# zju-vipa/ProtoPFormer

Hardware: AMD Instinct MI355X
Metric: images/sec train step, deit_small+2000 protos, bs256, 1/2/4/8 MI355X (higher is better)
Workload: dtype bf16; 1 GPU; deit_small_patch16_224, synthetic 224x224, 2000x384 prototypes, 200 classes, k=81, batch 256/GPU (BASELINE.json configs[2]), train step = fwd+CE+PPC+bwd+allreduce+AdamW+EMA, DropPath 0.1; blocks after the token reservation run compacted on the 1+k reserved rows (equal to the masked full-length blocks to bf16 rounding); bf16 backbone: the reserved tokens differ from the fp32 reference's in ~2-3 % o; global_batch=256, parallelism=dp1

## Files before the change

### include/ppf_hip.h

```cpp
#ifndef PPF_HIP_H
#define PPF_HIP_H

#include <stddef.h>
#include <stdint.h>

#ifdef __cplusplus
extern "C" {
#endif

typedef struct ihipStream_t* ppf_stream_t;

#define PPF_ERR_SHAPE (-1)
#define PPF_ERR_ALIGN (-2)
#define PPF_ERR_ARG (-3)

#define PPF_ABI_VERSION 10

const char* ppf_last_error(void);
int ppf_abi_version(void);
int ppf_device_info(int* cu_count, int* clock_mhz, char* name, int name_len);
int ppf_stream_arm(ppf_stream_t stream, int on);
int ppf_stream_wait_stream(ppf_stream_t dst, ppf_stream_t src);
int64_t ppf_stream_mark(ppf_stream_t stream);
int ppf_stream_wait_mark(ppf_stream_t stream, int64_t ticket);

int ppf_gemm_bf16(const void* A, const void* B, void* C, int M, int N, int K, int lda, int ldb, int ldc, int trans_a,
                  int trans_b, int epi, const float* bias, const float* res, int ldres, const float* rowscale,
                  int rows_per_group, const float* colscale, const void* aux_in, void* aux_out, int ldaux, float* colsum,
                  float alpha, void* workspace, size_t workspace_bytes, ppf_stream_t stream);
size_t ppf_gemm_workspace_bytes(int M, int N, int K);

int ppf_gemm_test_force_g224(int force);

int ppf_gemm_probe(int enable);
int ppf_gemm_probe_read(double* ms_total, int64_t* launches, double* flops, double* bytes);

int ppf_path_probe(int enable);
int ppf_path_probe_read(int tag, double* ms_total, int64_t* launches, double* flops, double* bytes);

int ppf_gemm_bf16_batched(const void* A, const void* B, void* C, int M, int N, int K, int lda, int ldb, int ldc, int trans_a,
                          int trans_b, int out_f32, float alpha, int batch_outer, int batch_inner, int64_t sa_o, int64_t sa_i,
                          int64_t sb_o, int64_t sb_i, int64_t sc_o, int64_t sc_i, int kpad, ppf_stream_t stream);

int ppf_layernorm_bwd_f32(const float* dy, const float* x, const int* row_map, const float* w, const float* dres_in, float* dx_out, float* dw, float* db,
                          int rows, int D, float eps, ppf_stream_t stream);
int ppf_ew_bwd_f32(int kind, const float* a, const float* b, float* out, const float* rowscale, int rows_per_group, int M, int N, ppf_stream_t stream);
int ppf_colsum_f32(const float* in, float* out, int M, int N, ppf_stream_t stream);
int ppf_attn_bwd_f32(const float* qkv, const float* dout, const float* policy, float* dqkv, float* scratch, int B, int H, int N, int D, int self_keep,
                     int eps_n, ppf_stream_t stream);
int ppf_th_attn_bwd_f32(const float* qkv, const float* dout, const float* wl, const float* bl, const float* ww, const float* bw, float* dqkv,
                        float* dwl, float* dbl, float* dww, float* dbw, int B, int H, int N, int D, ppf_stream_t stream);
int ppf_class_attn_bwd_f32(const float* q, const float* k, const float* v, const float* policy, const float* dout, float* dq, float* dk, float* dv,
                           int B, int H, int N1, int D, ppf_stream_t stream);

int ppf_rowgemm_supported(int D, int K, int rows_per_tile);
int ppf_rowgemm_bf16(const void* A, const void* B, int M, int D, int K, int lda, int ldb, int rows_per_tile, const float* bias, void* out,
                     ppf_stream_t stream);
int ppf_rowgemm_resid_ln(const void* A, const void* B, int M, int D, int K, int lda, int ldb, int rows_per_tile, const float* bias,
                         const float* res, float* xout, const float* rowscale, int rows_per_group, const float* colscale, void* aux_out,
                         const float* ln_w, const float* ln_b, void* ln_out, float* ln_mean, float* ln_rstd, float eps, ppf_stream_t stream);
int ppf_rowgemm_lnbwd(const void* A, const void* B, int M, int D, int K, int lda, int ldb, int rows_per_tile, const float* x, const float* mean,
                      const float* rstd, const float* w, const float* dres_in, float* dx_out, void* cast_out, const float* rowscale,
                      int rows_per_group, const float* colscale, const void* branch, float* partial, size_t partial_bytes, ppf_stream_t stream);
int ppf_rowgemm_colsum(const float* partial, int tiles, int D, int nparts, float* dw, float* db, float* dg, ppf_stream_t stream);
int ppf_transpose_bf16_batched(const void* src, void* dst, const void* desc_i64, int n, int total_tiles, ppf_stream_t stream);

int ppf_layernorm_fwd(const float* x, const int* row_map, const float* w, const float* b, void* y, float* mean, float* rstd,
                      int rows, int D, float eps, ppf_stream_t stream);
int ppf_layernorm_bwd(const void* dy, const float* x, const int* row_map, const float* w, const float* mean, const float* rstd,
                      const float* dres_in, float* dx_out, float* dw, float* db, void* cast_out, const float* rowscale,
                      int rows_per_group, const float* colscale, float* dbias_next, const void* branch, float* dcolscale,
                      int rows, int D, float* partial, size_t partial_bytes, ppf_stream_t stream);
int ppf_layernorm_bwd_blocks(int rows);
int ppf_layernorm_bwd_reduce(const float* partial, int rows, int D, float* dw, float* db, float* dbias_next, float* dcolscale,
                             ppf_stream_t stream);

int ppf_attn_fwd(const void* qkv, void* out, const float* policy, float* rowmax, float* zinv, int B, int H, int N, int D,
                 int self_keep, int eps_n, ppf_stream_t stream);
int ppf_attn_fwd_hm_supported(int H, int N, int D);
int ppf_attn_fwd_hm(const void* qkv, void* out, const float* policy, float* rowmax, float* zinv, float* headmean, int NP, int B, int H, int N,
                    int D, int self_keep, int eps_n, ppf_stream_t stream);
int ppf_attn_headmean(const void* qkv, const float* policy, const float* rowmax, const float* zinv, float* headmean, int NP,
                      int B, int H, int N, int D, int self_keep, int eps_n, ppf_stream_t stream);
int ppf_attn_bwd(const void* qkv, const void* out, const void* dout, void* dqkv, const float* policy, const float* rowmax,
                 const float* zinv, float* delta, int B, int H, int N, int D, int self_keep, int eps_n, ppf_stream_t stream);

int ppf_th_scores(const void* qkv, const float* wl, const float* bl, float* sp, int B, int H, int N, int D, int NP, ppf_stream_t stream);
int ppf_th_dwl(const void* qkv, const float* ds_prime, float* dwl, int B, int H, int N, int D, int NP, ppf_stream_t stream);
int ppf_th_softmax_mix(float* sp, void* a16, float* hm, const float* ww, const float* bw, int B, int H, int N, int NP, int NPK,
                       ppf_stream_t stream);
int ppf_th_softmax_bwd(const float* prob, float* da, void* ds16, const float* ww, const float* wl, float* dww, float* dbw, float* dbl,
                       int B, int H, int N, int NP, int NPK, ppf_stream_t stream);
int ppf_th_fused_supported(int H, int N, int D);
int ppf_th_fwd(const void* qkv, const float* wl, const float* bl, const float* ww, const float* bw, void* a16, float* hm, float* rowmax,
               float* zinv, void* out, int B, int H, int N, int D, int NP, int NPK, ppf_stream_t stream);
size_t ppf_th_bwd_partial_floats(int B, int H, int N);
int ppf_th_bwd(const void* qkv, const void* dout, const float* wl, const float* bl, const float* ww, const float* rowmax, const float* zinv,
               void* ds16, float* partial, int B, int H, int N, int D, int NPK, ppf_stream_t stream);
int ppf_th_param_reduce(const float* partial, int B, int H, int N, float* dww, float* dbw, float* dbl, float* dwl, ppf_stream_t stream);
int ppf_th_grads_supported(int H, int N, int D);
int ppf_th_grads(const void* qkv, const void* dout, const void* ds16, const void* a16, void* dqkv, int B, int H, int N, int D, int NPK,
                 ppf_stream_t stream);
int ppf_class_attn_fwd(const void* q, const void* k, const void* v, const float* policy, float* attn, float* zinv, float* rowmean,
                       void* out, int B, int H, int N1, int D, ppf_stream_t stream);
int ppf_class_attn_bwd(const void* q, const void* k, const void* v, const float* attn, const float* zinv, const void* dout, void* dq,
                       void* dk, void* dv, int B, int H, int N1, int D, ppf_stream_t stream);
int ppf_merge3_cast(const float* a, const float* b, const float* cq, void* out, int rows, int D, int N1, ppf_stream_t stream);

int ppf_rollout_threshold(const float* hm_layer, int B, int N, int NP, int kdrop, void* thr_out_u32, ppf_stream_t stream);
int ppf_rollout(const float* hm, int64_t layer_stride, int L, int B, int N, int NP, const float* init_rows, int n_init, int lead,
                int kdrop, int kdrop_init, float identity, int k, const void* thr_u32, float* cls_attn, int* idx, float* policy,
                ppf_stream_t stream);
int ppf_topk_sorted(const float* scores, int B, int n, int k, int* idx, ppf_stream_t stream);

int ppf_proto_fwd(const float* tok, int64_t stride_b, int t0, int T, const float* protos, int B, int P, int Dp, int act_kind,
// ... 122 lines not shown
```

### protopformer_amd/csrc/gemm_bf16.hip

```cpp
#include "ppf_common.h"
#include "ppf_hip.h"
#include "gemm_common.h"
#include <cstdlib>
#include <type_traits>

namespace {
using namespace ppfg;

constexpr int BM = 128, BN = 128, BK = 64, NTHREADS = 256;
constexpr int TILE_BYTES = BM * BK * 2;
constexpr int STAGE_LD = 68;
constexpr int STAGE_BYTES = 4 * 32 * STAGE_LD * 4;


__device__ __forceinline__ int lds_off_mode0(int r, int c16) { return lds_row_off(r, c16); }
template <int ROWS>
__device__ __forceinline__ int lds_off_mode1(int kc, int col) {
    return kc * (ROWS * 2) + ((((col >> 5) ^ (kc & 3))) << 6) + ((col & 31) << 1);
}

typedef uint32_t u32x4 __attribute__((ext_vector_type(4)));

template <bool T, int ROWS, int NTHR = NTHREADS>
struct TileIO {
    static constexpr int NLD = ROWS * 8 / NTHR;
    static constexpr int RPP = NTHR / 8;
    static constexpr int CPR = ROWS / 8;
    static constexpr int KPP = NTHR / CPR;
    static __device__ __forceinline__ unsigned gload(u32x4 (&reg)[NLD], const bf16_t* __restrict__ X, int ld, int R, int row0,
                                                     int k0, int kend, int tid, int kpad) {
        unsigned mask = 0;
        if constexpr (!T) {
            const int c16 = tid & 7, rb = tid >> 3;
            const bool kok = kpad ? (k0 + c16 * 8) < kend : (k0 + c16 * 8 + 8) <= kend;
            const int kk = kok ? k0 + c16 * 8 : 0;
#pragma unroll
            for (int i = 0; i < NLD; ++i) {
                const int r = row0 + rb + RPP * i;
                const bf16_t* src = X + (size_t)min(r, R - 1) * ld + kk;
                reg[i] = *reinterpret_cast<const u32x4*>(src);
                mask |= (kok && r < R) ? (1u << i) : 0u;
            }
        } else {
            const int c16 = tid % CPR, kb = tid / CPR;
            const int col = row0 + c16 * 8;
            const bool cok = kpad ? col < R : (col + 8) <= R;
            const int cc = cok ? col : 0;
#pragma unroll
            for (int i = 0; i < NLD; ++i) {
                const int kc = k0 + kb + KPP * i;
                const bf16_t* src = X + (size_t)min(kc, kend - 1) * ld + cc;
                reg[i] = *reinterpret_cast<const u32x4*>(src);
                mask |= (cok && kc < kend) ? (1u << i) : 0u;
            }
        }
        return mask;
    }
    static __device__ __forceinline__ void sstore(const u32x4 (&reg)[NLD], unsigned mask, unsigned char* tile, int tid) {
        const u32x4 zero = {0u, 0u, 0u, 0u};
        if constexpr (!T) {
            const int c16 = tid & 7, rb = tid >> 3;
#pragma unroll
            for (int i = 0; i < NLD; ++i)
                *reinterpret_cast<u32x4*>(tile + lds_off_mode0(rb + RPP * i, c16)) = ((mask >> i) & 1u) ? reg[i] : zero;
        } else {
            const int c16 = tid % CPR, kb = tid / CPR;
#pragma unroll
            for (int i = 0; i < NLD; ++i)
                *reinterpret_cast<u32x4*>(tile + lds_off_mode1<ROWS>(kb + KPP * i, c16 * 8)) = ((mask >> i) & 1u) ? reg[i] : zero;
        }
    }
    static __device__ __forceinline__ bf16x8 frag(const unsigned char* tile, int rbase, int ks, int lane) {
        if constexpr (!T) {
            return *reinterpret_cast<const bf16x8*>(tile + lds_off_mode0(rbase + (lane & 31), ks * 2 + (lane >> 5)));
        } else {
            typedef __attribute__((address_space(3))) bf16x4 lds_bf16x4;
            const int s = lane & 15, g16 = (lane >> 4) & 1, h = lane >> 5;
            const int col = rbase + 16 * g16 + 4 * (s & 3);
            const int kc = ks * 16 + 8 * h + (s >> 2);
            bf16x4 lo = __builtin_amdgcn_ds_read_tr16_b64_v4bf16((lds_bf16x4*)(tile + lds_off_mode1<ROWS>(kc, col)));
            bf16x4 hi = __builtin_amdgcn_ds_read_tr16_b64_v4bf16((lds_bf16x4*)(tile + lds_off_mode1<ROWS>(kc + 4, col)));
            return __builtin_shufflevector(lo, hi, 0, 1, 2, 3, 4, 5, 6, 7);
        }
    }
};


template <int EPI>
__device__ __forceinline__ void epilogue_rows(const GemmParams& p, const float* stage, int mbase, int nbase, int lane) {
    if (EpiWide<EPI>::value && ((p.ldc | p.ldaux) & 7) == 0) {
        const int col = (lane & 7) * 8;
        const int n = nbase + col;
        if (n + 8 <= p.N) {
            const EpiCols8 cc = epi_load_cols8<EPI>(p, n, true);
            EpiRow8 rr[4];
#pragma unroll
            for (int pass = 0; pass < 4; ++pass) {
                const int m = mbase + pass * 8 + (lane >> 3);
                rr[pass] = epi_load_row8<EPI>(p, m, n, m < p.M);
            }
#pragma unroll
            for (int pass = 0; pass < 4; ++pass) {
                const int r = pass * 8 + (lane >> 3);
                const int m = mbase + r;
                const float4 a = *reinterpret_cast<const float4*>(stage + r * STAGE_LD + col);
                const float4 b = *reinterpret_cast<const float4*>(stage + r * STAGE_LD + col + 4);
                if (m < p.M) epi_store8<EPI>(p, m, n, a, b, cc, rr[pass]);
            }
        } else if (n < p.N) {
            const EpiCols cc = epi_load_cols<EPI>(p, n, true);
#pragma unroll
            for (int pass = 0; pass < 4; ++pass) {
                const int r = pass * 8 + (lane >> 3);
                const int m = mbase + r;
                if (m < p.M) {
                    const EpiRow rr = epi_load_row<EPI>(p, m, n, true);
                    const float4 v = *reinterpret_cast<const float4*>(stage + r * STAGE_LD + col);
                    epi_store<EPI>(p, m, n, v.x, v.y, v.z, v.w, cc, rr);
                }
            }
        }
    } else {
        const int col = (lane & 15) * 4;
        const int n = nbase + col;
        const EpiCols cc = epi_load_cols<EPI>(p, n, n < p.N);
        EpiRow rr[8];
#pragma unroll
        for (int pass = 0; pass < 8; ++pass) {
            const int m = mbase + pass * 4 + (lane >> 4);
            rr[pass] = epi_load_row<EPI>(p, m, n, m < p.M && n < p.N);
        }
#pragma unroll
        for (int pass = 0; pass < 8; ++pass) {
            const int r = pass * 4 + (lane >> 4);
            const int m = mbase + r;
            const float4 v = *reinterpret_cast<const float4*>(stage + r * STAGE_LD + col);
            if (m < p.M && n < p.N) epi_store<EPI>(p, m, n, v.x, v.y, v.z, v.w, cc, rr[pass]);
        }
    }
}

struct KSlice { int kbeg, kend; };
__device__ __forceinline__ KSlice k_slice(int K, int nsplit, int zslice) {
    const int kchunk = (((K + nsplit - 1) / nsplit) + BK - 1) / BK * BK;
    const int kbeg = zslice * kchunk;
    return {kbeg, min(K, kbeg + kchunk)};
}

template <int EPI, int MT>
__device__ __forceinline__ void strip_epilogue(const GemmParams& p, const f32x16 (&acc)[2][MT], int mi, unsigned char* smem, int wave, int lane,
                                               int mbase, int nbase) {
    const int h = lane >> 5;
    float* stage = reinterpret_cast<float*>(smem) + wave * (32 * STAGE_LD);
#pragma unroll
    for (int ni = 0; ni < 2; ++ni)
#pragma unroll
        for (int g = 0; g < 4; ++g)
            *reinterpret_cast<float4*>(stage + (lane & 31) * STAGE_LD + 32 * ni + 8 * g + 4 * h) =
                make_float4(acc[ni][mi][4 * g], acc[ni][mi][4 * g + 1], acc[ni][mi][4 * g + 2], acc[ni][mi][4 * g + 3]);
    __builtin_amdgcn_wave_barrier();
    epilogue_rows<EPI>(p, stage, mbase, nbase, lane);
    __builtin_amdgcn_wave_barrier();
}

__device__ __forceinline__ void store_partial_colsum(const GemmParams& p, int m, float v) {
    p.ws[p.zslice * ((size_t)p.M * p.N + (size_t)p.cs_parts * p.M) + (size_t)p.M * p.N + m] = v;
}

template <bool TA, bool TB, int EPI, bool COLSUM>
__global__ __launch_bounds__(NTHREADS, 3) void gemm_kernel(const GemmParams p_) {
    constexpr int PD = 1, MT = 2;
    extern __shared__ __attribute__((aligned(16))) unsigned char smem[];
    constexpr int TBM = 64 * MT;
    constexpr int A_BYTES = TBM * BK * 2;
    using IOA = TileIO<TA, TBM>;
    using IOB = TileIO<TB, BN>;
    const int tid = threadIdx.x, lane = tid & 63, wave = tid >> 6;
    const int wm = (wave & 1) * (32 * MT), wn = (wave >> 1) * 64;

    const int tiles_n = (p_.N + BN - 1) / BN;
    const int tiles = tiles_n * ((p_.M + TBM - 1) / TBM);
    const int vid_all = xcd_remap(blockIdx.x, gridDim.x);
    const int zslice = vid_all / tiles, vid = vid_all - zslice * tiles;
    const int m0 = (vid / tiles_n) * TBM, n0 = (vid % tiles_n) * BN;
    GemmParams p = p_;
    p.zslice = zslice;
    if (gridDim.y > 1) {
        const int bo = blockIdx.y / p.batch_inner, bi = blockIdx.y % p.batch_inner;
        p.A += bo * p.sa_o + bi * p.sa_i;
        p.B += bo * p.sb_o + bi * p.sb_i;
        const long long co = bo * p.sc_o + bi * p.sc_i;
        p.C = (EPI == EPI_BF16) ? (void*)(reinterpret_cast<bf16_t*>(p.C) + co) : (void*)(reinterpret_cast<float*>(p.C) + co);
    }

    const auto [kbeg, kend] = k_slice(p.K, p.nsplit, zslice);
    if (kbeg >= kend) return;
    const int nk = (kend - kbeg + BK - 1) / BK;

    u32x4 ra[PD][IOA::NLD], rb[PD][IOB::NLD];
    unsigned ma[PD], mb[PD];
    f32x16 acc[2][MT];
#pragma unroll
    for (int i = 0; i < 2; ++i)
#pragma unroll
        for (int j = 0; j < MT; ++j)
#pragma unroll
            for (int r = 0; r < 16; ++r) acc[i][j][r] = 0.f;
    f32x16 accs[MT];
    if constexpr (COLSUM) {
#pragma unroll
        for (int j = 0; j < MT; ++j)
#pragma unroll
            for (int r = 0; r < 16; ++r) accs[j][r] = 0.f;
    }
    const bool do_colsum = COLSUM && p.colsum != nullptr && n0 == 0 && wn == 0;
    unsigned char* tA = smem;
    unsigned char* tB = smem + A_BYTES;

#pragma unroll
    for (int st = 0; st < PD; ++st) {
        const int k0 = min(kbeg + st * BK, kbeg + (nk - 1) * BK);
        ma[st] = IOA::gload(ra[st], p.A, p.lda, p.M, m0, k0, kend, tid, p.kpad);
        mb[st] = IOB::gload(rb[st], p.B, p.ldb, p.N, n0, k0, kend, tid, p.kpad);
    }
    IOA::sstore(ra[0], ma[0], tA, tid);
    IOB::sstore(rb[0], mb[0], tB, tid);
    __syncthreads();

    for (int kt0 = 0; kt0 < nk; kt0 += PD) {
#pragma unroll
        for (int u = 0; u < PD; ++u) {
            const int kt = kt0 + u;
            if (kt >= nk) break;
            {
                const int k0 = kbeg + min(kt + PD, nk - 1) * BK;
                ma[u] = IOA::gload(ra[u], p.A, p.lda, p.M, m0, k0, kend, tid, p.kpad);
                mb[u] = IOB::gload(rb[u], p.B, p.ldb, p.N, n0, k0, kend, tid, p.kpad);
            }
#pragma unroll
            for (int ks = 0; ks < BK / 16; ++ks) {
                bf16x8 fa[MT], fb[2];
#pragma unroll
                for (int i = 0; i < MT; ++i) fa[i] = IOA::frag(tA, wm + 32 * i, ks, lane);
#pragma unroll
                for (int i = 0; i < 2; ++i) fb[i] = IOB::frag(tB, wn + 32 * i, ks, lane);
#pragma unroll
                for (int ni = 0; ni < 2; ++ni)
#pragma unroll
                    for (int mi = 0; mi < MT; ++mi)
                        acc[ni][mi] = __builtin_amdgcn_mfma_f32_32x32x16_bf16(fb[ni], fa[mi], acc[ni][mi], 0, 0, 0);
                if constexpr (COLSUM) {
                    if (do_colsum) {
                        bf16x8 ones;
#pragma unroll
                        for (int e = 0; e < 8; ++e) ones[e] = (__bf16)1.0f;
#pragma unroll
                        for (int mi = 0; mi < MT; ++mi)
                            accs[mi] = __builtin_amdgcn_mfma_f32_32x32x16_bf16(ones, fa[mi], accs[mi], 0, 0, 0);
                    }
                }
            }
            __syncthreads();
            if (kt + 1 < nk) {
                IOA::sstore(ra[(u + 1) % PD], ma[(u + 1) % PD], tA, tid);
                IOB::sstore(rb[(u + 1) % PD], mb[(u + 1) % PD], tB, tid);
            }
            __syncthreads();
        }
    }

#pragma unroll
    for (int mi = 0; mi < MT; ++mi) {
        strip_epilogue<EPI>(p, acc, mi, smem, wave, lane, m0 + wm + 32 * mi, n0 + wn);
        if constexpr (COLSUM) {
            const int m = m0 + wm + 32 * mi + (lane & 31);
            if (do_colsum && (lane >> 5) == 0 && m < p.M) {
                if constexpr (EPI == EPI_PARTIAL) store_partial_colsum(p, m, accs[mi][0]);
                else unsafeAtomicAdd(p.colsum + m, accs[mi][0]);
            }
        }
    }
}

template <int WMW, int WNW, bool COLSUM>
__global__ __launch_bounds__(64 * WMW * WNW, 1) void wgrad8_kernel(const GemmParams p_) {
    extern __shared__ __attribute__((aligned(16))) unsigned char smem[];
    constexpr int NTHR = 64 * WMW * WNW, TBM = 64 * WMW, TBN = 64 * WNW;
    using IOA = TileIO<true, TBM, NTHR>;
    using IOB = TileIO<true, TBN, NTHR>;
    const int tid = threadIdx.x, lane = tid & 63;
    const int wave = __builtin_amdgcn_readfirstlane(tid >> 6);
    const int wm = (wave % WMW) * 64, wn = (wave / WMW) * 64;
    const int tiles_n = (p_.N + TBN - 1) / TBN;
    const int tiles = tiles_n * ((p_.M + TBM - 1) / TBM);
    const int vid_all = xcd_remap(blockIdx.x, gridDim.x);
    const int zslice = vid_all / tiles, vid = vid_all - zslice * tiles;
    const int m0 = (vid / tiles_n) * TBM, n0 = (vid % tiles_n) * TBN;
    GemmParams p = p_;
    p.zslice = zslice;
    const auto [kbeg, kend] = k_slice(p.K, p.nsplit, zslice);
    if (kbeg >= kend) return;
    const int nk = (kend - kbeg + BK - 1) / BK;

    u32x4 ra[IOA::NLD], rb[IOB::NLD];
    unsigned ma, mb;
    f32x16 acc[2][2];
#pragma unroll
    for (int i = 0; i < 2; ++i)
#pragma unroll
        for (int j = 0; j < 2; ++j)
#pragma unroll
            for (int r = 0; r < 16; ++r) acc[i][j][r] = 0.f;
    f32x16 accs[2];
    if constexpr (COLSUM) {
#pragma unroll
        for (int j = 0; j < 2; ++j)
#pragma unroll
            for (int r = 0; r < 16; ++r) accs[j][r] = 0.f;
    }
    const bool do_colsum = COLSUM && p.colsum != nullptr && n0 == 0 && wn == 0;
    unsigned char* tA = smem;
    unsigned char* tB = smem + TBM * BK * 2;
    ma = IOA::gload(ra, p.A, p.lda, p.M, m0, kbeg, kend, tid, 0);
    mb = IOB::gload(rb, p.B, p.ldb, p.N, n0, kbeg, kend, tid, 0);
    IOA::sstore(ra, ma, tA, tid);
    IOB::sstore(rb, mb, tB, tid);
    __syncthreads();
    for (int kt = 0; kt < nk; ++kt) {
        {
            const int k0 = kbeg + min(kt + 1, nk - 1) * BK;
            ma = IOA::gload(ra, p.A, p.lda, p.M, m0, k0, kend, tid, 0);
            mb = IOB::gload(rb, p.B, p.ldb, p.N, n0, k0, kend, tid, 0);
        }
#pragma unroll
        for (int ks = 0; ks < BK / 16; ++ks) {
            bf16x8 fa[2], fb[2];
#pragma unroll
            for (int i = 0; i < 2; ++i) fa[i] = IOA::frag(tA, wm + 32 * i, ks, lane);
#pragma unroll
            for (int i = 0; i < 2; ++i) fb[i] = IOB::frag(tB, wn + 32 * i, ks, lane);
#pragma unroll
            for (int ni = 0; ni < 2; ++ni)
#pragma unroll
                for (int mi = 0; mi < 2; ++mi) acc[ni][mi] = __builtin_amdgcn_mfma_f32_32x32x16_bf16(fb[ni], fa[mi], acc[ni][mi], 0, 0, 0);
            if constexpr (COLSUM) {
                if (do_colsum) {
                    bf16x8 ones;
#pragma unroll
                    for (int e = 0; e < 8; ++e) ones[e] = (__bf16)1.0f;
#pragma unroll
                    for (int mi = 0; mi < 2; ++mi) accs[mi] = __builtin_amdgcn_mfma_f32_32x32x16_bf16(ones, fa[mi], accs[mi], 0, 0, 0);
                }
            }
        }
        __syncthreads();
        if (kt + 1 < nk) {
            IOA::sstore(ra, ma, tA, tid);
            IOB::sstore(rb, mb, tB, tid);
        }
        __syncthreads();
    }
#pragma unroll
    for (int mi = 0; mi < 2; ++mi) {
        strip_epilogue<EPI_PARTIAL>(p, acc, mi, smem, wave, lane, m0 + wm + 32 * mi, n0 + wn);
        if constexpr (COLSUM) {
            const int m = m0 + wm + 32 * mi + (lane & 31);
            if (do_colsum && (lane >> 5) == 0 && m < p.M) store_partial_colsum(p, m, accs[mi][0]);
        }
    }
}

template <int WMW, int WNW>
int launch_wgrad8(const GemmParams& p, int splitk, hipStream_t stream) {
    constexpr int NTHR = 64 * WMW * WNW, TBM = 64 * WMW, TBN = 64 * WNW;
    constexpr int opnd = (TBM + TBN) * BK * 2, strips = (NTHR / 64) * 32 * STAGE_LD * 4;
    constexpr int lds = opnd > strips ? opnd : strips;
    const int tiles = ((p.M + TBM - 1) / TBM) * ((p.N + TBN - 1) / TBN);
    return ppf_launch<wgrad8_kernel<WMW, WNW, true>>(dim3(tiles * splitk), dim3(NTHR), lds, stream, "wgrad8", p);
}

typedef __attribute__((address_space(3))) void g4_lds_t;
typedef const __attribute__((address_space(1))) void g4_gbl_t;

template <int NLA>
struct DirectLds {
    unsigned offA[NLA], offB[4];
    const unsigned char *gA, *gB;
    __device__ __forceinline__ DirectLds(const GemmParams& p, int m0, int n0, int tid)
        : gA(reinterpret_cast<const unsigned char*>(p.A)), gB(reinterpret_cast<const unsigned char*>(p.B)) {
        const int rb = tid >> 3, ch = (tid & 7) ^ lds_swz(rb);
#pragma unroll
        for (int i = 0; i < NLA; ++i) offA[i] = ((unsigned)min(m0 + rb + 32 * i, p.M - 1) * (unsigned)p.lda + ch * 8) * 2u;
#pragma unroll
        for (int i = 0; i < 4; ++i) offB[i] = ((unsigned)min(n0 + rb + 32 * i, p.N - 1) * (unsigned)p.ldb + ch * 8) * 2u;
    }
    __device__ __forceinline__ void load(int kt, unsigned char* tA, unsigned char* tB, int wave) const {
        const unsigned char* ka = gA + (size_t)kt * (BK * 2);
        const unsigned char* kb = gB + (size_t)kt * (BK * 2);
#pragma unroll
        for (int i = 0; i < NLA; ++i)
            __builtin_amdgcn_global_load_lds((g4_gbl_t*)(ka + offA[i]), (g4_lds_t*)(tA + i * 4096 + wave * 1024), 16, 0, 0);
#pragma unroll
        for (int i = 0; i < 4; ++i)
            __builtin_amdgcn_global_load_lds((g4_gbl_t*)(kb + offB[i]), (g4_lds_t*)(tB + i * 4096 + wave * 1024), 16, 0, 0);
        asm volatile("s_waitcnt vmcnt(0)" ::: "memory");
        __syncthreads();
    }
};

template <int EPI>
__global__ __launch_bounds__(NTHREADS, 4) void gemm128g_kernel(const GemmParams p) {
    extern __shared__ __attribute__((aligned(16))) unsigned char smem[];
    using IO = TileIO<false, 128>;
    const int tid = threadIdx.x, lane = tid & 63;
    const int wave = __builtin_amdgcn_readfirstlane(tid >> 6);
    const int wm = (wave & 1) * 64, wn = (wave >> 1) * 64;
    const int tiles_n = (p.N + BN - 1) / BN;
    const int vid = xcd_remap(blockIdx.x, gridDim.x);
    const int m0 = (vid / tiles_n) * BM, n0 = (vid % tiles_n) * BN;
    unsigned char* tA = smem;
    unsigned char* tB = smem + TILE_BYTES;
    const DirectLds<BM / 32> dl(p, m0, n0, tid);
    f32x16 acc[2][2];
#pragma unroll
    for (int i = 0; i < 2; ++i)
#pragma unroll
        for (int j = 0; j < 2; ++j)
#pragma unroll
            for (int r = 0; r < 16; ++r) acc[i][j][r] = 0.f;

    const int nk = p.K / BK;
    for (int kt = 0; kt < nk; ++kt) {
        if (kt > 0) __syncthreads();
        dl.load(kt, tA, tB, wave);
#pragma unroll
        for (int ks = 0; ks < BK / 16; ++ks) {
            bf16x8 fa[2], fb[2];
#pragma unroll
            for (int i = 0; i < 2; ++i) fa[i] = IO::frag(tA, wm + 32 * i, ks, lane);
#pragma unroll
            for (int i = 0; i < 2; ++i) fb[i] = IO::frag(tB, wn + 32 * i, ks, lane);
#pragma unroll
            for (int ni = 0; ni < 2; ++ni)
#pragma unroll
                for (int mi = 0; mi < 2; ++mi)
                    acc[ni][mi] = __builtin_amdgcn_mfma_f32_32x32x16_bf16(fb[ni], fa[mi], acc[ni][mi], 0, 0, 0);
        }
    }
    __syncthreads();
#pragma unroll
    for (int mi = 0; mi < 2; ++mi) strip_epilogue<EPI>(p, acc, mi, smem, wave, lane, m0 + wm + 32 * mi, n0 + wn);
}

template <int EPI>
int launch_g4(const GemmParams& p, hipStream_t stream) {
    constexpr int lds = 2 * TILE_BYTES > STAGE_BYTES ? 2 * TILE_BYTES : STAGE_BYTES;
    const int tiles = ((p.M + BM - 1) / BM) * ((p.N + BN - 1) / BN);
    return ppf_launch<gemm128g_kernel<EPI>>(dim3(tiles), dim3(NTHREADS), lds, stream, "gemm128g", p);
}

constexpr int G224_ROWS = 224, G224_MT = 7, G224_LD = 36;
// ... 49 lines not shown
                                                                                 pack_bf16x2(b.x * p.alpha, b.y * p.alpha), pack_bf16x2(b.z * p.alpha, b.w * p.alpha));
        }
        __builtin_amdgcn_fence(__ATOMIC_RELEASE, "wavefront");
        __builtin_amdgcn_wave_barrier();
    }
}

bool g4_eligible(const GemmParams& p);
int g_force_g224 = 0;
bool g224_eligible(const GemmParams& p, int epi) {
    if (epi != EPI_BF16 || p.bias != nullptr || p.kpad || p.K % BK != 0 || p.N % 8 != 0 || (p.ldc & 7) != 0) return false;
    if ((long long)p.M * p.lda >= (1ll << 30) || (long long)p.N * p.ldb >= (1ll << 30)) return false;
    if (g_force_g224) return true;
    if (p.K < 768) return false;
    const int cus = ppf_cu_count();
    const long long tn = (p.N + BN - 1) / BN;
    const long long t128 = (long long)((p.M + BM - 1) / BM) * tn, t224 = (long long)((p.M + G224_ROWS - 1) / G224_ROWS) * tn;
    const int per128 = g4_eligible(p) ? 4 : 3;
    auto cost = [](long long tiles, long long slots, int rows, int per) {
        const long long full = tiles / slots, rest = tiles - full * slots;
        double c = (double)full * rows * per;
        if (rest) c += rows * per * (4 * rest >= slots ? 1.0 : 0.5);
        return c;
    };
    return t128 >= (long long)per128 * cus && cost(t224, 3ll * cus, G224_ROWS, 3) < 0.97 * cost(t128, (long long)per128 * cus, BM, per128);
}
int launch_g224(const GemmParams& p, hipStream_t stream) {
    constexpr int lds = G224_ROWS * BK * 2 + TILE_BYTES;
    const int tiles = ((p.M + G224_ROWS - 1) / G224_ROWS) * ((p.N + BN - 1) / BN);
    return ppf_launch<gemm224g_kernel>(dim3(tiles), dim3(NTHREADS), lds, stream, "gemm224g", p);
}

bool g4_eligible(const GemmParams& p) {
    return p.K % BK == 0 && p.K <= 512 && p.N >= 512 && !p.kpad && (long long)p.M * p.lda < (1ll << 30) &&
           (long long)p.N * p.ldb < (1ll << 30) && (long long)((p.M + BM - 1) / BM) * ((p.N + BN - 1) / BN) >= 512;
}

template <bool TA, bool TB, int EPI, bool COLSUM>
int launch(const GemmParams& p, int splitk, hipStream_t stream, int nbatch = 1) {
    const int tiles = ((p.M + BM - 1) / BM) * ((p.N + BN - 1) / BN);
    constexpr int lds = 2 * TILE_BYTES > STAGE_BYTES ? 2 * TILE_BYTES : STAGE_BYTES;
    GemmParams q = p;
    q.nsplit = splitk;
    return ppf_launch<gemm_kernel<TA, TB, EPI, COLSUM>>(dim3(tiles * splitk, nbatch, 1), dim3(NTHREADS), lds, stream, "gemm", q);
}

__global__ __launch_bounds__(256) void splitk_reduce_kernel(const float* __restrict__ ws, float* __restrict__ C, float* __restrict__ colsum,
                                                            int M, int N, int ldc, int nsplit, int cs_parts) {
    const size_t mn = (size_t)M * N, slice = mn + (colsum ? (size_t)cs_parts * M : 0);
    const size_t total4 = mn / 4;
    const size_t i = (size_t)blockIdx.x * 256 + threadIdx.x;
    if (i < total4) {
        const float* p = ws + i * 4;
        float4 acc = make_float4(0.f, 0.f, 0.f, 0.f);
        for (int z0 = 0; z0 < nsplit; z0 += 16) {
            float4 v[16];
#pragma unroll
            for (int u = 0; u < 16; ++u) {
                const int z = min(z0 + u, nsplit - 1);
                v[u] = *reinterpret_cast<const float4*>(p + (size_t)z * slice);
            }
#pragma unroll
            for (int u = 0; u < 16; ++u)
                if (z0 + u < nsplit) { acc.x += v[u].x; acc.y += v[u].y; acc.z += v[u].z; acc.w += v[u].w; }
        }
        const size_t e = i * 4, m = e / N, n = e - m * N;
        float4* dst = reinterpret_cast<float4*>(C + m * ldc + n);
        const float4 c = *dst;
        *dst = make_float4(c.x + acc.x, c.y + acc.y, c.z + acc.z, c.w + acc.w);
    } else if (colsum && i < total4 + (size_t)M) {
        const size_t m = i - total4;
        float a = 0.f;
        for (int z = 0; z < nsplit; ++z)
            for (int q = 0; q < cs_parts; ++q) a += ws[(size_t)z * slice + mn + (size_t)q * M + m];
        colsum[m] += a;
    }
}

PpfEventPool g_probe;
bool g_probe_on = false;

constexpr size_t PPF_GEMM_COUNTER_BYTES = 16384;

int pick_splitk(int M, int N, int K) {
    const int tiles = ((M + BM - 1) / BM) * ((N + BN - 1) / BN);
    const int target = min(M, N) <= 256 ? 216 : 432;
    int s = target / tiles;
    const int maxs = (K + 4 * BK - 1) / (4 * BK);
    if (s > maxs) s = maxs;
    if (s < 1) s = 1;
    const int kchunk = (((K + s - 1) / s) + BK - 1) / BK * BK;
    return (K + kchunk - 1) / kchunk;
}

template <int... EPIS, class F>
bool dispatch_epi(int epi, int& rc, F&& f) {
    return ((epi == EPIS && (rc = f(std::integral_constant<int, EPIS>()), true)) || ...);
}

}

extern "C" {

int ppf_gemm_test_force_g224(int force) { g_force_g224 = force != 0; return 0; }

size_t ppf_gemm_workspace_bytes(int M, int N, int K) {
    return PPF_GEMM_COUNTER_BYTES + (size_t)pick_splitk(M, N, K) * ((size_t)M * N + M) * sizeof(float);
}

int ppf_gemm_bf16(const void* A, const void* B, void* C, int M, int N, int K, int lda, int ldb, int ldc, int trans_a,
                  int trans_b, int epi, const float* bias, const float* res, int ldres, const float* rowscale,
                  int rows_per_group, const float* colscale, const void* aux_in, void* aux_out, int ldaux, float* colsum,
                  float alpha, void* workspace, size_t workspace_bytes, hipStream_t stream) {
    PPF_CHECK_ARG(M > 0 && N > 0 && K > 0, PPF_ERR_SHAPE, "ppf_gemm_bf16: bad shape M=%d N=%d K=%d", M, N, K);
    PPF_CHECK_ARG((lda % 8) == 0 && (ldb % 8) == 0 && (ldc % 4) == 0 && (N % 4) == 0, PPF_ERR_ALIGN,
                  "ppf_gemm_bf16: lda/ldb must be multiples of 8, ldc and N of 4 (lda=%d ldb=%d ldc=%d N=%d)", lda, ldb, ldc, N);
    PPF_CHECK_ARG(trans_a ? (M % 8 == 0) : (K % 8 == 0), PPF_ERR_ALIGN, "ppf_gemm_bf16: A inner extent must be a multiple of 8");
    PPF_CHECK_ARG(trans_b ? (N % 8 == 0) : (K % 8 == 0), PPF_ERR_ALIGN, "ppf_gemm_bf16: B inner extent must be a multiple of 8");
    PPF_CHECK_ARG((((uintptr_t)A | (uintptr_t)B | (uintptr_t)C) & 15) == 0, PPF_ERR_ALIGN, "ppf_gemm_bf16: pointers must be 16-byte aligned");
    PPF_CHECK_ARG(!(trans_a && !trans_b), PPF_ERR_ARG, "ppf_gemm_bf16: (trans_a=1, trans_b=0) is not instantiated");
    PPF_CHECK_ARG((((uintptr_t)aux_in | (uintptr_t)aux_out | (uintptr_t)res) & 15) == 0 && (ldaux % 4) == 0 && (ldres % 4) == 0, PPF_ERR_ALIGN,
                  "ppf_gemm_bf16: aux / residual pointers must be 16-byte aligned, ldaux and ldres multiples of 4 (the epilogues use 8/16-byte accesses)");
    GemmParams p;
    p.A = (const bf16_t*)A; p.B = (const bf16_t*)B; p.C = C; p.M = M; p.N = N; p.K = K; p.lda = lda; p.ldb = ldb; p.ldc = ldc;
    p.bias = bias; p.res = res; p.ldres = ldres; p.rowscale = rowscale; p.rows_per_group = rows_per_group > 0 ? rows_per_group : 1;
    p.colscale = colscale; p.aux_in = (const bf16_t*)aux_in; p.aux_out = (bf16_t*)aux_out; p.ldaux = ldaux; p.colsum = colsum; p.alpha = alpha; p.ws = nullptr;
    p.batch_inner = 1; p.sa_o = p.sa_i = p.sb_o = p.sb_i = p.sc_o = p.sc_i = 0; p.kpad = 0; p.cs_parts = 1; p.nsplit = 1;
    if (epi == EPI_RESID) PPF_CHECK_ARG(res != nullptr, PPF_ERR_ARG, "ppf_gemm_bf16: epi=4 needs a residual");
    if (epi == EPI_GELU) PPF_CHECK_ARG(aux_out != nullptr, PPF_ERR_ARG, "ppf_gemm_bf16: epi=2 needs aux_out");
    if (epi == EPI_DGELU) PPF_CHECK_ARG(aux_in != nullptr, PPF_ERR_ARG, "ppf_gemm_bf16: epi=5 needs aux_in");
    int rc;
    if (!trans_a && !trans_b) {
        if (g224_eligible(p, epi)) return launch_g224(p, stream);
        const auto g4 = [&](auto e) { return launch_g4<decltype(e)::value>(p, stream); };
        const auto nt = [&](auto e) { return launch<false, false, decltype(e)::value, false>(p, 1, stream); };
        if (g4_eligible(p) && dispatch_epi<EPI_BF16, EPI_GELU, EPI_RESID, EPI_DGELU>(epi, rc, g4)) return rc;
        if (dispatch_epi<EPI_BF16, EPI_F32, EPI_GELU, EPI_SIGMOID_F32, EPI_RESID, EPI_DGELU>(epi, rc, nt)) return rc;
    } else if (!trans_a && trans_b) {
        const auto nn = [&](auto e) { return launch<false, true, decltype(e)::value, false>(p, 1, stream); };
        if (dispatch_epi<EPI_BF16, EPI_F32, EPI_DGELU>(epi, rc, nn)) return rc;
    } else if (epi == EPI_ATOMIC) {
        const int ns = pick_splitk(M, N, K);
        const size_t need = PPF_GEMM_COUNTER_BYTES + (size_t)ns * ((size_t)M * N + M) * sizeof(float);
        if (workspace == nullptr || workspace_bytes < need || ns == 1) return launch<true, true, EPI_ATOMIC, true>(p, ns, stream);
        p.ws = (float*)((unsigned char*)workspace + PPF_GEMM_COUNTER_BYTES);
        p.cs_parts = 1;
        p.nsplit = ns;
        hipEvent_t e1 = nullptr;
        if (g_probe_on) {
            const auto ev = g_probe.acquire();
            (void)hipEventRecord(ev.first, stream);
            e1 = ev.second;
        }
        const bool wide = (M < N ? M : N) >= 320;
        if (wide && M >= 512 && M >= N && (M % 256 == 0 || M >= 1024)) rc = launch_wgrad8<4, 2>(p, ns, stream);
        else if (wide && N >= 512 && (N % 256 == 0 || N >= 1024)) rc = launch_wgrad8<2, 4>(p, ns, stream);
        else rc = launch<true, true, EPI_PARTIAL, true>(p, ns, stream);
        if (rc) return rc;
        if (e1) {
            (void)hipEventRecord(e1, stream);
            g_probe.flops += 2.0 * M * N * (double)K;
            g_probe.bytes += 2.0 * ((double)M * K + (double)N * K) + 4.0 * M * N;
        }
        const size_t work = (size_t)M * N / 4 + (colsum ? M : 0);
        const int grid = (int)((work + 255) / 256);
        hipLaunchKernelGGL(splitk_reduce_kernel, dim3(grid), dim3(256), 0, stream, p.ws, (float*)C, colsum, M, N, ldc, ns, p.cs_parts);
        PPF_LAUNCH_CHECK();
        return 0;
    } else if (epi == EPI_F32) {
        return launch<true, true, EPI_F32, false>(p, 1, stream);
    }
    ppf_set_error("ppf_gemm_bf16: combination trans_a=%d trans_b=%d epi=%d not instantiated", trans_a, trans_b, epi);
    return PPF_ERR_ARG;
}

int ppf_gemm_probe(int enable) {
    if (enable == 1) g_probe.reset();
    if (enable == 2) g_probe.destroy();
    g_probe_on = enable == 1;
    return 0;
}
int ppf_gemm_probe_read(double* ms_total, int64_t* launches, double* flops, double* bytes) {
    return g_probe.sum_ms("ppf_gemm_probe_read", ms_total, launches, flops, bytes);
}

int ppf_gemm_bf16_batched(const void* A, const void* B, void* C, int M, int N, int K, int lda, int ldb, int ldc, int trans_a, int trans_b,
                          int out_f32, float alpha, int batch_outer, int batch_inner, int64_t sa_o, int64_t sa_i, int64_t sb_o, int64_t sb_i,
// ... 32 lines not shown
```

Measured before the change: 17230 images/sec.

## Stream wgrad8 operand tiles into a double-buffered LDS ring via direct-to-LDS DMA

Adds a DMA variant of the weight-gradient GEMM kernel that loads A/B tiles straight from global memory into LDS with a two-slot ring. It spreads the next tile's issues across the k-steps of the current tile and double-buffers the MFMA fragments. The goal is to remove the register round-trip and one of the two barriers per k-tile in the old gload/sstore path. It is on by default when K is a multiple of BK, with a test hook to force either path, and it needs more LDS (a 96KB ring), which limits occupancy.

```diff
diff --git a/include/ppf_hip.h b/include/ppf_hip.h
--- a/include/ppf_hip.h
+++ b/include/ppf_hip.h
@@ -31,6 +31,7 @@
 size_t ppf_gemm_workspace_bytes(int M, int N, int K);
 
 int ppf_gemm_test_force_g224(int force);
+int ppf_gemm_test_wgrad_path(int path);
 
 int ppf_gemm_probe(int enable);
 int ppf_gemm_probe_read(double* ms_total, int64_t* launches, double* flops, double* bytes);
diff --git a/protopformer_amd/csrc/gemm_bf16.hip b/protopformer_amd/csrc/gemm_bf16.hip
--- a/protopformer_amd/csrc/gemm_bf16.hip
+++ b/protopformer_amd/csrc/gemm_bf16.hip
@@ -1,23 +1,20 @@
 #include "ppf_common.h"
 #include "ppf_hip.h"
 #include "gemm_common.h"
+#include "gemm_layout.h"
 #include <cstdlib>
 #include <type_traits>
 
 namespace {
 using namespace ppfg;
 
-constexpr int BM = 128, BN = 128, BK = 64, NTHREADS = 256;
+constexpr int BM = 128, BN = 128, NTHREADS = 256;
 constexpr int TILE_BYTES = BM * BK * 2;
 constexpr int STAGE_LD = 68;
 constexpr int STAGE_BYTES = 4 * 32 * STAGE_LD * 4;
 
 
 __device__ __forceinline__ int lds_off_mode0(int r, int c16) { return lds_row_off(r, c16); }
-template <int ROWS>
-__device__ __forceinline__ int lds_off_mode1(int kc, int col) {
-    return kc * (ROWS * 2) + ((((col >> 5) ^ (kc & 3))) << 6) + ((col & 31) << 1);
-}
 
 typedef uint32_t u32x4 __attribute__((ext_vector_type(4)));
 
@@ -140,13 +137,6 @@
     }
 }
 
-struct KSlice { int kbeg, kend; };
-__device__ __forceinline__ KSlice k_slice(int K, int nsplit, int zslice) {
-    const int kchunk = (((K + nsplit - 1) / nsplit) + BK - 1) / BK * BK;
-    const int kbeg = zslice * kchunk;
-    return {kbeg, min(K, kbeg + kchunk)};
-}
-
 template <int EPI, int MT>
 __device__ __forceinline__ void strip_epilogue(const GemmParams& p, const f32x16 (&acc)[2][MT], int mi, unsigned char* smem, int wave, int lane,
                                                int mbase, int nbase) {
@@ -282,7 +272,27 @@
     }
 }
 
-template <int WMW, int WNW, bool COLSUM>
+#ifndef WG8_ISSUE_REGIONS
+#define WG8_ISSUE_REGIONS 3
+#endif
+template <bool COLSUM>
+__device__ __forceinline__ void wgrad8_mma(const bf16x8 (&fa)[2], const bf16x8 (&fb)[2], f32x16 (&acc)[2][2], f32x16 (&accs)[2], bool do_colsum) {
+#pragma unroll
+    for (int ni = 0; ni < 2; ++ni)
+#pragma unroll
+        for (int mi = 0; mi < 2; ++mi) acc[ni][mi] = __builtin_amdgcn_mfma_f32_32x32x16_bf16(fb[ni], fa[mi], acc[ni][mi], 0, 0, 0);
+    if constexpr (COLSUM) {
+        if (do_colsum) {
+            bf16x8 ones;
+#pragma unroll
+            for (int e = 0; e < 8; ++e) ones[e] = (__bf16)1.0f;
+#pragma unroll
+            for (int mi = 0; mi < 2; ++mi) accs[mi] = __builtin_amdgcn_mfma_f32_32x32x16_bf16(ones, fa[mi], accs[mi], 0, 0, 0);
+        }
+    }
+}
+
+template <int WMW, int WNW, bool COLSUM, bool DMA>
 __global__ __launch_bounds__(64 * WMW * WNW, 1) void wgrad8_kernel(const GemmParams p_) {
     extern __shared__ __attribute__((aligned(16))) unsigned char smem[];
     constexpr int NTHR = 64 * WMW * WNW, TBM = 64 * WMW, TBN = 64 * WNW;
@@ -302,8 +312,6 @@
     if (kbeg >= kend) return;
     const int nk = (kend - kbeg + BK - 1) / BK;
 
-    u32x4 ra[IOA::NLD], rb[IOB::NLD];
-    unsigned ma, mb;
     f32x16 acc[2][2];
 #pragma unroll
     for (int i = 0; i < 2; ++i)
@@ -319,45 +327,98 @@
             for (int r = 0; r < 16; ++r) accs[j][r] = 0.f;
     }
     const bool do_colsum = COLSUM && p.colsum != nullptr && n0 == 0 && wn == 0;
-    unsigned char* tA = smem;
-    unsigned char* tB = smem + TBM * BK * 2;
-    ma = IOA::gload(ra, p.A, p.lda, p.M, m0, kbeg, kend, tid, 0);
-    mb = IOB::gload(rb, p.B, p.ldb, p.N, n0, kbeg, kend, tid, 0);
-    IOA::sstore(ra, ma, tA, tid);
-    IOB::sstore(rb, mb, tB, tid);
-    __syncthreads();
-    for (int kt = 0; kt < nk; ++kt) {
-        {
-            const int k0 = kbeg + min(kt + 1, nk - 1) * BK;
-            ma = IOA::gload(ra, p.A, p.lda, p.M, m0, k0, kend, tid, 0);
-            mb = IOB::gload(rb, p.B, p.ldb, p.N, n0, k0, kend, tid, 0);
-        }
-#pragma unroll
-        for (int ks = 0; ks < BK / 16; ++ks) {
-            bf16x8 fa[2], fb[2];
-#pragma unroll
-            for (int i = 0; i < 2; ++i) fa[i] = IOA::frag(tA, wm + 32 * i, ks, lane);
-#pragma unroll
-            for (int i = 0; i < 2; ++i) fb[i] = IOB::frag(tB, wn + 32 * i, ks, lane);
-#pragma unroll
-            for (int ni = 0; ni < 2; ++ni)
-#pragma unroll
-                for (int mi = 0; mi < 2; ++mi) acc[ni][mi] = __builtin_amdgcn_mfma_f32_32x32x16_bf16(fb[ni], fa[mi], acc[ni][mi], 0, 0, 0);
-            if constexpr (COLSUM) {
-                if (do_colsum) {
-                    bf16x8 ones;
-#pragma unroll
-                    for (int e = 0; e < 8; ++e) ones[e] = (__bf16)1.0f;
-#pragma unroll
-                    for (int mi = 0; mi < 2; ++mi) accs[mi] = __builtin_amdgcn_mfma_f32_32x32x16_bf16(ones, fa[mi], accs[mi], 0, 0, 0);
+    constexpr int A_BYTES = TBM * BK * 2;
+    if constexpr (!DMA) {
+        u32x4 ra[IOA::NLD], rb[IOB::NLD];
+        unsigned ma, mb;
+        unsigned char* tA = smem;
+        unsigned char* tB = smem + A_BYTES;
+        ma = IOA::gload(ra, p.A, p.lda, p.M, m0, kbeg, kend, tid, 0);
+        mb = IOB::gload(rb, p.B, p.ldb, p.N, n0, kbeg, kend, tid, 0);
+        IOA::sstore(ra, ma, tA, tid);
+        IOB::sstore(rb, mb, tB, tid);
+        __syncthreads();
+        for (int kt = 0; kt < nk; ++kt) {
+            {
+                const int k0 = kbeg + min(kt + 1, nk - 1) * BK;
+                ma = IOA::gload(ra, p.A, p.lda, p.M, m0, k0, kend, tid, 0);
+                mb = IOB::gload(rb, p.B, p.ldb, p.N, n0, k0, kend, tid, 0);
+            }
+#pragma unroll
+            for (int ks = 0; ks < BK / 16; ++ks) {
+                bf16x8 fa[2], fb[2];
+#pragma unroll
+                for (int i = 0; i < 2; ++i) fa[i] = IOA::frag(tA, wm + 32 * i, ks, lane);
+#pragma unroll
+                for (int i = 0; i < 2; ++i) fb[i] = IOB::frag(tB, wn + 32 * i, ks, lane);
+                wgrad8_mma<COLSUM>(fa, fb, acc, accs, do_colsum);
+            }
+            __syncthreads();
+            if (kt + 1 < nk) {
+                IOA::sstore(ra, ma, tA, tid);
+                IOB::sstore(rb, mb, tB, tid);
+            }
+            __syncthreads();
+        }
+    } else {
+        constexpr int NPA = TBM / 8, NPB = TBN / 8, PPW = (NPA + NPB) / 8;
+        static_assert(NTHR == 512 && A_BYTES + TBN * BK * 2 == WG8_SLOT_BYTES && NPA % 8 == 0, "ring slot layout");
+        const unsigned offA = (unsigned)(wgrad_dma_src(wgrad_dma_piece<TBM>(wave, lane), 0, p.lda, m0, p.M) * 2);
+        const unsigned offB = (unsigned)(wgrad_dma_src(wgrad_dma_piece<TBN>(wave, lane), 0, p.ldb, n0, p.N) * 2);
+        const size_t stepA = (size_t)p.lda * (BK * 2), stepB = (size_t)p.ldb * (BK * 2);
+        const size_t pieceA = (size_t)p.lda * (4096 / TBM * 2), pieceB = (size_t)p.ldb * (4096 / TBN * 2);
+        const unsigned char* gA = reinterpret_cast<const unsigned char*>(p.A) + (size_t)kbeg * p.lda * 2;
+        const unsigned char* gB = reinterpret_cast<const unsigned char*>(p.B) + (size_t)kbeg * p.ldb * 2;
+        const uint32_t ring = __builtin_amdgcn_readfirstlane(lds_offset_of(smem)) + wave * 1024;
+        auto issue = [&](int i, uint32_t dst) __attribute__((always_inline)) {
+            if (8 * i < NPA) lds_dma16_hidden(gA + i * pieceA + offA, dst + 8192 * i);
+            else lds_dma16_hidden(gB + (i - NPA / 8) * pieceB + offB, dst + 8192 * i);
+        };
+
+        auto tile = [&](const unsigned char* st, uint32_t nxt, auto issue_tag) __attribute__((always_inline)) {
+            constexpr bool ISSUE = decltype(issue_tag)::value;
+            constexpr int NKS = BK / 16, NRI = WG8_ISSUE_REGIONS;
+            const unsigned char* tA = st;
+            const unsigned char* tB = st + A_BYTES;
+            bf16x8 fa[2][2], fb[2][2];
+#pragma unroll
+            for (int i = 0; i < 2; ++i) fa[0][i] = IOA::frag(tA, wm + 32 * i, 0, lane);
+#pragma unroll
+            for (int i = 0; i < 2; ++i) fb[0][i] = IOB::frag(tB, wn + 32 * i, 0, lane);
+#pragma unroll
+            for (int ks = 0; ks < NKS; ++ks) {
+                __builtin_amdgcn_sched_barrier(0);
+                if constexpr (ISSUE) {
+                    if (ks < NRI) {
+#pragma unroll
+                        for (int k = ks * PPW / NRI; k < (ks + 1) * PPW / NRI; ++k) issue(k, nxt);
+                    }
                 }
-            }
-        }
-        __syncthreads();
-        if (kt + 1 < nk) {
-            IOA::sstore(ra, ma, tA, tid);
-            IOB::sstore(rb, mb, tB, tid);
-        }
+                if (ks + 1 < NKS) {
+#pragma unroll
+                    for (int i = 0; i < 2; ++i) fa[(ks + 1) & 1][i] = IOA::frag(tA, wm + 32 * i, ks + 1, lane);
+#pragma unroll
+                    for (int i = 0; i < 2; ++i) fb[(ks + 1) & 1][i] = IOB::frag(tB, wn + 32 * i, ks + 1, lane);
+                }
+                wgrad8_mma<COLSUM>(fa[ks & 1], fb[ks & 1], acc, accs, do_colsum);
+            }
+            __builtin_amdgcn_sched_barrier(0);
+        };
+
+#pragma unroll
+        for (int i = 0; i < PPW; ++i) issue(i, ring);
+        int slot = 0;
+        for (int kt = 0; kt + 1 < nk; ++kt) {
+            asm volatile("s_waitcnt vmcnt(0)" ::: "memory");
+            __builtin_amdgcn_s_barrier();
+            gA += stepA;
+            gB += stepB;
+            tile(smem + slot * WG8_SLOT_BYTES, ring + (slot ^ 1) * WG8_SLOT_BYTES, std::true_type());
+            slot ^= 1;
+        }
+        asm volatile("s_waitcnt vmcnt(0)" ::: "memory");
+        __builtin_amdgcn_s_barrier();
+        tile(smem + slot * WG8_SLOT_BYTES, 0u, std::false_type());
         __syncthreads();
     }
 #pragma unroll
@@ -370,13 +431,24 @@
     }
 }
 
+int g_wgrad_path = 0;
+#ifndef PPF_WGRAD_DMA_DEFAULT
+#define PPF_WGRAD_DMA_DEFAULT 1
+#endif
+bool wgrad8_dma(const GemmParams& p) {
+    if (p.K % BK != 0 || g_wgrad_path == 1) return false;
+    return g_wgrad_path == 2 || PPF_WGRAD_DMA_DEFAULT;
+}
+
 template <int WMW, int WNW>
 int launch_wgrad8(const GemmParams& p, int splitk, hipStream_t stream) {
     constexpr int NTHR = 64 * WMW * WNW, TBM = 64 * WMW, TBN = 64 * WNW;
     constexpr int opnd = (TBM + TBN) * BK * 2, strips = (NTHR / 64) * 32 * STAGE_LD * 4;
     constexpr int lds = opnd > strips ? opnd : strips;
+    static_assert(strips <= WG8_RING_BYTES, "the epilogue strips reuse the dead ring");
     const int tiles = ((p.M + TBM - 1) / TBM) * ((p.N + TBN - 1) / TBN);
-    return ppf_launch<wgrad8_kernel<WMW, WNW, true>>(dim3(tiles * splitk), dim3(NTHR), lds, stream, "wgrad8", p);
+    if (wgrad8_dma(p)) return ppf_launch<wgrad8_kernel<WMW, WNW, true, true>>(dim3(tiles * splitk), dim3(NTHR), WG8_RING_BYTES, stream, "wgrad8 (dma)", p);
+    return ppf_launch<wgrad8_kernel<WMW, WNW, true, false>>(dim3(tiles * splitk), dim3(NTHR), lds, stream, "wgrad8", p);
 }
 
 typedef __attribute__((address_space(3))) void g4_lds_t;
@@ -592,16 +664,6 @@
 
 constexpr size_t PPF_GEMM_COUNTER_BYTES = 16384;
 
-int pick_splitk(int M, int N, int K) {
-    const int tiles = ((M + BM - 1) / BM) * ((N + BN - 1) / BN);
-    const int target = min(M, N) <= 256 ? 216 : 432;
-    int s = target / tiles;
-    const int maxs = (K + 4 * BK - 1) / (4 * BK);
-    if (s > maxs) s = maxs;
-    if (s < 1) s = 1;
-    const int kchunk = (((K + s - 1) / s) + BK - 1) / BK * BK;
-    return (K + kchunk - 1) / kchunk;
-}
 
 template <int... EPIS, class F>
 bool dispatch_epi(int epi, int& rc, F&& f) {
@@ -613,6 +675,12 @@
 extern "C" {
 
 int ppf_gemm_test_force_g224(int force) { g_force_g224 = force != 0; return 0; }
+
+int ppf_gemm_test_wgrad_path(int path) {
+    PPF_CHECK_ARG(path >= 0 && path <= 2, PPF_ERR_ARG, "ppf_gemm_test_wgrad_path: path must be 0, 1 or 2 (got %d)", path);
+    g_wgrad_path = path;
+    return 0;
+}
 
 size_t ppf_gemm_workspace_bytes(int M, int N, int K) {
     return PPF_GEMM_COUNTER_BYTES + (size_t)pick_splitk(M, N, K) * ((size_t)M * N + M) * sizeof(float);
diff --git a/protopformer_amd/csrc/gemm_layout.h b/protopformer_amd/csrc/gemm_layout.h
--- /dev/null
+++ b/protopformer_amd/csrc/gemm_layout.h
@@ -0,0 +1,54 @@
+#pragma once
+#include <stddef.h>
+
+#if defined(__HIPCC__)
+#define PPF_HD __host__ __device__ __forceinline__
+#else
+#define PPF_HD inline
+#endif
+
+namespace ppfg {
+
+constexpr int BK = 64;
+
+template <int ROWS>
+PPF_HD int lds_off_mode1(int kc, int col) {
+    return kc * (ROWS * 2) + ((((col >> 5) ^ (kc & 3))) << 6) + ((col & 31) << 1);
+}
+
+struct KSlice { int kbeg, kend; };
+PPF_HD KSlice k_slice(int K, int nsplit, int zslice) {
+    const int kchunk = (((K + nsplit - 1) / nsplit) + BK - 1) / BK * BK;
+    const int kbeg = zslice * kchunk;
+    return {kbeg, K < kbeg + kchunk ? K : kbeg + kchunk};
+}
+
+#ifndef PPF_WGRAD_SPLITK_TARGET
+#define PPF_WGRAD_SPLITK_TARGET 432
+#endif
+inline int pick_splitk(int M, int N, int K) {
+    const int tiles = ((M + 127) / 128) * ((N + 127) / 128);
+    const int target = (M < N ? M : N) <= 256 ? 216 : PPF_WGRAD_SPLITK_TARGET;
+    int s = target / tiles;
+    const int maxs = (K + 4 * BK - 1) / (4 * BK);
+    if (s > maxs) s = maxs;
+    if (s < 1) s = 1;
+    const int kchunk = (((K + s - 1) / s) + BK - 1) / BK * BK;
+    return (K + kchunk - 1) / kchunk;
+}
+
+constexpr int WG8_SLOT_BYTES = (256 + 128) * BK * 2;
+constexpr int WG8_RING_BYTES = 2 * WG8_SLOT_BYTES;
+struct DmaPiece { int kc, col, lds; };
+template <int ROWS>
+PPF_HD DmaPiece wgrad_dma_piece(int piece, int lane) {
+    const int lds = piece * 1024 + lane * 16;
+    const int kc = lds / (ROWS * 2), w = lds % (ROWS * 2);
+    return {kc, ((((w >> 6) ^ (kc & 3))) << 5) + ((w & 63) >> 1), lds};
+}
+PPF_HD size_t wgrad_dma_src(const DmaPiece& pc, int k0, int ld, int row0, int R) {
+    const int c = row0 + pc.col;
+    return (size_t)(k0 + pc.kc) * (size_t)ld + (size_t)(c < R - 8 ? c : R - 8);
+}
+
+}
```

Measured after the change: 17450 images/sec, median of 6. +1.3%, better.
